# netty/netty

Hardware: AMD Instinct MI355X
Metric: GiB/s device-resident Snappy encode+decode, 64 KiB chunks, 1/2/4/8 MI355X (higher is better)
Workload: dtype u8; 1 GPU; configs[4]: Snappy encode (+frame CRC32C) then decode + CRC32C verify of 1638400 text-like 64 KiB chunks (100 GiB) split across 1 GPU(s), device-resident; chunk_bytes=65536, global_chunks=1638400, chunks_per_gpu=1638400, parallelism=dp1 (independent chunk shards, no data-path collective)

## Files before the change

### netty_amd/csrc/snappy_encode.hip

```cpp
#include <stdlib.h>
#include <algorithm>
#include <mutex>
#include <vector>
#include "nx_common.hpp"
#include "workspace.hpp"

namespace nx {
namespace enc {

typedef uint32_t __attribute__((aligned(1))) u32u;

typedef uint64_t __attribute__((aligned(1))) u64u;

__device__ __forceinline__ uint32_t ld32(const uint8_t* p) { return *reinterpret_cast<const u32u*>(p); }
__device__ __forceinline__ uint64_t ld64(const uint8_t* p) { return *reinterpret_cast<const u64u*>(p); }
__device__ __forceinline__ uint32_t hash_of(uint32_t le, int shift) {
    return (__builtin_bswap32(le) * 0x1e35a7bdu) >> shift;
}

template <bool PAIR>
struct WriterT {
    uint32_t* w;
    uint32_t acc;
    uint32_t na;
    uint32_t nw;
    uint32_t s0;
    __device__ __forceinline__ void emit(uint32_t v) {
        if (!PAIR) {
            w[nw] = v;
        } else if (nw & 1u) {
            *reinterpret_cast<uint2*>(w + nw - 1u) = make_uint2(s0, v);
        } else {
            s0 = v;
        }
        ++nw;
    }
    __device__ __forceinline__ void put(uint32_t b) {
        acc |= b << (8 * na);
        if (++na == 4) {
            emit(acc);
            acc = 0;
            na = 0;
        }
    }
    __device__ __forceinline__ void copy(const uint8_t* p, int32_t n) {
        while (n >= 4) {
            const uint32_t v = ld32(p);
            if (na == 0) {
                emit(v);
            } else {
                emit(acc | (v << (8 * na)));
                acc = v >> (32 - 8 * na);
            }
            p += 4;
            n -= 4;
        }
        while (n-- > 0) put(*p++);
    }
    __device__ __forceinline__ uint32_t pos() const { return nw * 4 + na; }
    __device__ __forceinline__ void finish() {
        if (PAIR && (nw & 1u)) w[nw - 1u] = s0;
        uint8_t* t = reinterpret_cast<uint8_t*>(w + nw);
        for (uint32_t i = 0; i < na; ++i) t[i] = (uint8_t)(acc >> (8 * i));
    }
};

template <int SD>
struct WriterL {
    uint32_t* st;
    uint32_t* dst;
    uint32_t acc;
    uint32_t na;
    uint32_t nw;
    uint32_t s;
    uint32_t lo;
    __device__ __forceinline__ WriterL(uint32_t* stage, uint8_t* o)
        : st(stage), dst(reinterpret_cast<uint32_t*>(o)), acc(0), na(0), nw(0) {
        s = (uint32_t)(((uintptr_t)o >> 2) & (SD - 1));
        lo = s;
    }
    __device__ __forceinline__ void emit(uint32_t v) {
        st[s] = v;
        ++nw;
        if (s == SD - 1) {
            uint32_t* g = dst + nw - SD;
            if (lo == 0) {
#pragma unroll
                for (int q = 0; q < SD / 4; ++q)
                    reinterpret_cast<uint4*>(g)[q] = make_uint4(st[4 * q], st[4 * q + 1], st[4 * q + 2], st[4 * q + 3]);
            } else {
                for (uint32_t j = lo; j < SD; ++j) g[j] = st[j];
                lo = 0;
            }
            s = 0;
        } else {
            ++s;
        }
    }
    __device__ __forceinline__ void put(uint32_t b) {
        acc |= b << (8 * na);
        if (++na == 4) {
            emit(acc);
            acc = 0;
            na = 0;
        }
    }
    __device__ __forceinline__ void copy(const uint8_t* p, int32_t n) {
        while (n >= 4) {
            const uint32_t v = ld32(p);
            if (na == 0) {
                emit(v);
            } else {
                emit(acc | (v << (8 * na)));
                acc = v >> (32 - 8 * na);
            }
            p += 4;
            n -= 4;
        }
        while (n-- > 0) put(*p++);
    }
    __device__ __forceinline__ uint32_t pos() const { return nw * 4 + na; }
    __device__ __forceinline__ void finish() {
        uint32_t* g = dst + nw - s;
        for (uint32_t j = lo; j < s; ++j) g[j] = st[j];
        uint8_t* t = reinterpret_cast<uint8_t*>(dst + nw);
        for (uint32_t i = 0; i < na; ++i) t[i] = (uint8_t)(acc >> (8 * i));
    }
};

struct ByteWriter {
    uint8_t* o;
    uint32_t n;
    __device__ __forceinline__ void put(uint32_t b) { o[n++] = (uint8_t)b; }
    __device__ __forceinline__ void copy(const uint8_t* p, int32_t k) {
        for (int32_t i = 0; i < k; ++i) o[n + i] = p[i];
        n += (uint32_t)k;
    }
    __device__ __forceinline__ uint32_t pos() const { return n; }
    __device__ __forceinline__ void finish() {}
};

template <class Wr>
__device__ __forceinline__ void enc_literal(const uint8_t* in, Wr& w, int32_t length) {
    if (length < 61) {
        w.put((uint32_t)((length - 1) << 2));
    } else {
        const int32_t v = length - 1;
        const int bitLength = 31 - __clz((uint32_t)v);
        const int bytesToEncode = 1 + bitLength / 8;
        w.put((uint32_t)((59 + bytesToEncode) << 2));
        for (int i = 0; i < bytesToEncode; i++) w.put((uint32_t)((v >> (i * 8)) & 0xff));
    }
    w.copy(in, length);
}

template <class Wr>
__device__ __forceinline__ void enc_copy_off(Wr& w, int32_t offset, int32_t length) {
    if (length < 12 && offset < 2048) {
        w.put((uint32_t)(1 | ((length - 4) << 2) | ((offset >> 8) << 5)));
        w.put((uint32_t)(offset & 0xff));
    } else {
        w.put((uint32_t)(2 | ((length - 1) << 2)));
        w.put((uint32_t)(offset & 0xff));
        w.put((uint32_t)((offset >> 8) & 0xff));
    }
}

template <class Wr>
__device__ __forceinline__ void enc_copy(Wr& w, int32_t offset, int32_t length) {
    while (length >= 68) {
        enc_copy_off(w, offset, 64);
        length -= 64;
    }
    if (length > 64) {
        enc_copy_off(w, offset, 60);
        length -= 60;
    }
    enc_copy_off(w, offset, length);
}

struct StreamWin {
    const uint8_t* origin;
    uint32_t pad;
    uint32_t end;
    uint32_t wb;
    uint32_t w0, w1, w2, w3, w4, w5, w6, w7;
    uint32_t f0, f1, f2, f3;
    __device__ __forceinline__ void init(const uint8_t* in, int32_t length) {
        pad = (uint32_t)((uintptr_t)in & 15u);
        origin = in - pad;
        end = pad + (uint32_t)length;
        wb = 0x80000000u;
    }
    __device__ __forceinline__ static uint32_t sel(uint32_t i, uint32_t a0, uint32_t a1, uint32_t a2, uint32_t a3, uint32_t a4,
                                                   uint32_t a5, uint32_t a6, uint32_t a7) {
        const bool b0 = i & 1u, b1 = i & 2u, b2 = i & 4u;
        const uint32_t c0 = b0 ? a1 : a0, c1 = b0 ? a3 : a2, c2 = b0 ? a5 : a4, c3 = b0 ? a7 : a6;
        const uint32_t d0 = b1 ? c1 : c0, d1 = b1 ? c3 : c2;
        return b2 ? d1 : d0;
    }
    __device__ __forceinline__ uint32_t get(int32_t p) {
        const uint32_t q = (uint32_t)p + pad;
        uint32_t off = q - wb;
        if (off > 27u) {
            if (off < 44u) {
                wb += 16u;
                w0 = w4; w1 = w5; w2 = w6; w3 = w7;
                w4 = f0; w5 = f1; w6 = f2; w7 = f3;
                if (wb + 32u < end) {
                    const uint4 z = *reinterpret_cast<const uint4*>(origin + wb + 32u);
                    f0 = z.x; f1 = z.y; f2 = z.z; f3 = z.w;
                }
            } else {
                wb = q & ~15u;
                const uint4 x = *reinterpret_cast<const uint4*>(origin + wb);
                w0 = x.x; w1 = x.y; w2 = x.z; w3 = x.w;
                if (wb + 16u < end) {
                    const uint4 y = *reinterpret_cast<const uint4*>(origin + wb + 16u);
                    w4 = y.x; w5 = y.y; w6 = y.z; w7 = y.w;
                }
                if (wb + 32u < end) {
                    const uint4 z = *reinterpret_cast<const uint4*>(origin + wb + 32u);
                    f0 = z.x; f1 = z.y; f2 = z.z; f3 = z.w;
                }
            }
            off = q - wb;
        }
        const uint32_t i = off >> 2;
        const uint32_t lo = sel(i, w0, w1, w2, w3, w4, w5, w6, w7);
        const uint32_t hi = sel(i + 1u, w0, w1, w2, w3, w4, w5, w6, w7);
        return __builtin_amdgcn_alignbyte(hi, lo, off & 3u);
    }
};

__device__ __forceinline__ uint64_t ld_cand(const uint8_t* in, int32_t c, int32_t length) {
    return c + 8 <= length ? ld64(in + c) : (uint64_t)ld32(in + c);
}

__device__ __forceinline__ int32_t match_len(const uint8_t* in, StreamWin& win, int32_t a, int32_t b, int32_t length,
                                             uint32_t first) {
    int32_t m = 0;
    if (b <= length - 4) {
        const uint32_t x0 = first ^ win.get(b);
        if (x0) return (int32_t)(__builtin_ctz(x0) >> 3);
        m = 4;
        while (b + m <= length - 4) {
            const uint32_t x = ld32(in + a + m) ^ win.get(b + m);
            if (x) return m + (int32_t)(__builtin_ctz(x) >> 3);
            m += 4;
        }
    }
    while (b + m < length && in[a + m] == in[b + m]) ++m;
    return m;
}

template <bool SWAP, class Wr>
__device__ uint32_t encode_chunk(const uint8_t* __restrict__ in, int32_t length, Wr& w, uint32_t* __restrict__ table, uint32_t stamp) {
    for (int i = 0;; i++) {
        const uint32_t b = (uint32_t)length >> (i * 7);
        if ((b & 0xFFFFFF80u) != 0) {
            w.put((b & 0x7f) | 0x80);
        } else {
            w.put(b);
            break;
        }
    }
    uint32_t hts = length <= 1 ? 1u : (1u << (32 - __clz((uint32_t)(length - 1))));
    if (hts > 16384u) hts = 16384u;
    const int shift = __clz(hts) + 1;
    const uint32_t stag = stamp << 28;
    const uint32_t word0 = length >= 4 ? ld32(in) : 0u;
#define TST(ptr, v) (*(ptr) = (v))
#define XCH(ptr, v) (SWAP ? __hip_atomic_exchange((ptr), (v), __ATOMIC_RELAXED, __HIP_MEMORY_SCOPE_AGENT) \
                          : ({ const uint32_t o_ = *(ptr); *(ptr) = (v); o_; }))
#define CHK(wd) (((wd) ^ ((wd) >> 12) ^ ((wd) >> 24)) & 0xFFFu)
#define MK(pos, wd) (stag | (CHK(wd) << 16) | (uint32_t)(pos))
#define LIVE(e) (((e) & 0xF0000000u) == stag)
#define TBL_DEC(e) (LIVE(e) ? (int32_t)((e) & 0xFFFFu) : 0)
#define MAYBE(e, wd) (LIVE(e) ? ((((e) >> 16) & 0xFFFu) == CHK(wd)) : ((wd) == word0))
    int32_t nextEmit = 0;
    if (length >= 15) {
        StreamWin win;
        win.init(in, length);
        int32_t inIndex = 1;
        uint32_t nextWord = win.get(1);
        uint32_t nextHash = hash_of(nextWord, shift);
        for (;;) {
            int32_t skip = 32;
            int32_t nextIndex = inIndex;
            int32_t candidate;
            uint32_t curWord;
            uint64_t cand8;
            uint32_t entry;
            do {
                inIndex = nextIndex;
                const uint32_t hash = nextHash;
                curWord = nextWord;
                nextIndex = inIndex + (skip++ >> 5);
                if (nextIndex > length - 4) goto done;
                nextWord = win.get(nextIndex);
                nextHash = hash_of(nextWord, shift);
                entry = XCH(table + hash, MK(inIndex, curWord));
                candidate = TBL_DEC(entry);
            } while (!(MAYBE(entry, curWord) && curWord == (uint32_t)(cand8 = ld_cand(in, candidate, length))));

            enc_literal(in + nextEmit, w, inIndex - nextEmit);

            int32_t insertTail;
            for (;;) {
                const int32_t base = inIndex;
                const int32_t matched = 4 + match_len(in, win, candidate + 4, inIndex + 4, length, (uint32_t)(cand8 >> 32));
                inIndex += matched;
                enc_copy(w, base - candidate, matched);
                insertTail = inIndex - 1;
                nextEmit = inIndex;
                if (inIndex >= length - 4) goto done;
                const uint32_t wTail = win.get(insertTail);
                const uint32_t wCur = win.get(inIndex);
                const uint32_t prevHash = hash_of(wTail, shift);
                TST(table + prevHash, MK(inIndex - 1, wTail));
                const uint32_t currentHash = hash_of(wCur, shift);
                const uint32_t e = XCH(table + currentHash, MK(inIndex, wCur));
                candidate = TBL_DEC(e);
                if (!MAYBE(e, wCur) || wCur != (uint32_t)(cand8 = ld_cand(in, candidate, length))) break;
            }
            nextWord = win.get(insertTail + 2);
            nextHash = hash_of(nextWord, shift);
            ++inIndex;
        }
    }
done:
#undef TBL_DEC
#undef MAYBE
#undef LIVE
#undef MK
#undef CHK
#undef XCH
#undef TST
    if (nextEmit < length) enc_literal(in + nextEmit, w, length - nextEmit);
    w.finish();
    return w.pos();
}

__device__ __forceinline__ uint32_t bytes_at(const uint8_t* in, int32_t p, int32_t length) {
    if (p + 4 <= length) return ld32(in + p);
    uint32_t v = 0;
    for (int32_t i = 0; p + i < length && i < 4; ++i) v |= (uint32_t)in[p + i] << (8 * i);
    return v;
}

__device__ __forceinline__ int32_t match_len_w(const uint8_t* in, StreamWin& win, int32_t a, int32_t b, int32_t length, uint32_t cn3) {
    int32_t m = 0;
    if (b <= length - 4) {
        const uint32_t x0 = (cn3 ^ win.get(b)) & 0xFFFFFFu;
        if (x0) return (int32_t)(__builtin_ctz(x0) >> 3);
        m = 3;
        while (b + m <= length - 4) {
            const uint32_t x = ld32(in + a + m) ^ win.get(b + m);
            if (x) return m + (int32_t)(__builtin_ctz(x) >> 3);
            m += 4;
        }
    }
    while (b + m < length && in[a + m] == in[b + m]) ++m;
    return m;
}

template <class Wr>
__device__ uint32_t encode_chunk_w(const uint8_t* __restrict__ in, int32_t length, Wr& w, uint64_t* __restrict__ table, uint32_t stamp) {
    for (int i = 0;; i++) {
        const uint32_t b = (uint32_t)length >> (i * 7);
        if ((b & 0xFFFFFF80u) != 0) {
            w.put((b & 0x7f) | 0x80);
        } else {
            w.put(b);
            break;
        }
    }
    uint32_t hts = length <= 1 ? 1u : (1u << (32 - __clz((uint32_t)(length - 1))));
    if (hts > 16384u) hts = 16384u;
    const int shift = __clz(hts) + 1;
    int32_t nextEmit = 0;
    if (length >= 15) {
        const uint32_t pbits = hts == 16384u ? 16u : (uint32_t)(32 - shift);
        const uint32_t pmask = (1u << pbits) - 1u, rmask = (1u << shift) - 1u;
        const uint64_t stag = (uint64_t)stamp << 58;
        const uint32_t word0 = ld32(in);
        const uint32_t n3_0 = bytes_at(in, 4, length) & 0xFFFFFFu;
#define RES(wd) ((__builtin_bswap32(wd) * 0x1e35a7bdu) & rmask)
#define MKW(pos, wd, n3) (stag | ((uint64_t)(n3) << 34) | ((uint64_t)RES(wd) << pbits) | (uint64_t)(uint32_t)(pos))
#define WLIVE(e) ((uint32_t)((e) >> 58) == stamp)
#define WMATCH(e, wd) (WLIVE(e) ? (((uint32_t)((e) >> pbits) & rmask) == RES(wd)) : ((wd) == word0))
#define WPOS(e) (WLIVE(e) ? (int32_t)((uint32_t)(e) & pmask) : 0)
#define WN3(e) (WLIVE(e) ? ((uint32_t)((e) >> 34) & 0xFFFFFFu) : n3_0)
#define XCH64(ptr, v) __hip_atomic_exchange((ptr), (v), __ATOMIC_RELAXED, __HIP_MEMORY_SCOPE_AGENT)
        StreamWin win;
        win.init(in, length);
        int32_t inIndex = 1;
        uint32_t nextWord = win.get(1);
        uint32_t nextHash = hash_of(nextWord, shift);
        for (;;) {
            int32_t skip = 32;
            int32_t nextIndex = inIndex;
            uint64_t entry;
            uint32_t curWord;
            do {
                inIndex = nextIndex;
                const uint32_t hash = nextHash;
                curWord = nextWord;
                nextIndex = inIndex + (skip++ >> 5);
                if (nextIndex > length - 4) goto done;
                const uint32_t n3 = win.get(inIndex + 4) & 0xFFFFFFu;
                nextWord = win.get(nextIndex);
                nextHash = hash_of(nextWord, shift);
                entry = XCH64(table + hash, MKW(inIndex, curWord, n3));
            } while (!WMATCH(entry, curWord));
            int32_t candidate = WPOS(entry);
            uint32_t cn3 = WN3(entry);

            enc_literal(in + nextEmit, w, inIndex - nextEmit);

            int32_t insertTail;
            for (;;) {
                const int32_t base = inIndex;
                const int32_t matched = 4 + match_len_w(in, win, candidate + 4, inIndex + 4, length, cn3);
                inIndex += matched;
                enc_copy(w, base - candidate, matched);
                insertTail = inIndex - 1;
                nextEmit = inIndex;
                if (inIndex >= length - 4) goto done;
                const uint32_t wTail = win.get(insertTail);
                const uint32_t wCur = win.get(inIndex);
                const uint32_t n3c = win.get(inIndex + 4) & 0xFFFFFFu;
                const uint32_t n3t = ((wCur >> 24) | (n3c << 8)) & 0xFFFFFFu;
                const uint32_t prevHash = hash_of(wTail, shift);
                __hip_atomic_store(table + prevHash, MKW(inIndex - 1, wTail, n3t), __ATOMIC_RELAXED, __HIP_MEMORY_SCOPE_AGENT);
                const uint32_t currentHash = hash_of(wCur, shift);
                const uint64_t e = XCH64(table + currentHash, MKW(inIndex, wCur, n3c));
                if (!WMATCH(e, wCur)) break;
                candidate = WPOS(e);
                cn3 = WN3(e);
            }
            nextWord = win.get(insertTail + 2);
            nextHash = hash_of(nextWord, shift);
            ++inIndex;
        }
#undef XCH64
#undef WN3
#undef WPOS
#undef WMATCH
#undef WLIVE
#undef MKW
#undef RES
    }
done:
    if (nextEmit < length) enc_literal(in + nextEmit, w, length - nextEmit);
    w.finish();
    return w.pos();
}

constexpr int kStageDw = 16;
template <bool SWAP, bool SPREAD>
__global__ void __launch_bounds__(256, 5) k_snappy_encode(const uint8_t* __restrict__ in, const uint64_t* __restrict__ in_off,
                                                       const uint32_t* __restrict__ in_len, uint8_t* __restrict__ out,
                                                       const uint64_t* __restrict__ out_off, uint32_t* __restrict__ out_len,
                                                       int32_t* __restrict__ status, uint32_t n, uint64_t* __restrict__ workspace,
                                                       uint32_t stamp_base) {
    const uint32_t gtid = blockIdx.x * blockDim.x + threadIdx.x;
    if (SPREAD && (gtid & 63u) != 0u) return;
    const uint32_t tid = SPREAD ? gtid >> 6 : gtid;
    const uint32_t nthreads = SPREAD ? (gridDim.x * blockDim.x) >> 6 : gridDim.x * blockDim.x;
    uint64_t* table = workspace + (size_t)tid * 16384u;
    uint32_t* stage = nullptr;
    if constexpr (!SPREAD) {
        __shared__ uint32_t stages[256 * (kStageDw + 1)];
        stage = &stages[threadIdx.x * (kStageDw + 1)];
    }
    uint32_t iter = 0;
    for (uint32_t c = tid; c < n; c += nthreads, ++iter) {
        const uint32_t len = in_len[c];
        if (len > 65536u) {
            status[c] = NX_ERR_INVALID_ARG;
            out_len[c] = 0;
            continue;
        }
        const uint32_t stamp = stamp_base + iter + 1u;
        uint8_t* o = out + out_off[c];
        uint32_t olen;
        const uint8_t* src = in + in_off[c];
        if (!SPREAD && (((uintptr_t)o) & 3u) == 0) {
            WriterL<kStageDw> w(stage, o);
            olen = encode_chunk_w(src, (int32_t)len, w, table, stamp);
        } else if ((((uintptr_t)o) & 7u) == 0) {
            WriterT<true> w{reinterpret_cast<uint32_t*>(o), 0, 0, 0, 0};
            olen = encode_chunk_w(src, (int32_t)len, w, table, stamp);
        } else if ((((uintptr_t)o) & 3u) == 0) {
            WriterT<false> w{reinterpret_cast<uint32_t*>(o), 0, 0, 0, 0};
            olen = encode_chunk_w(src, (int32_t)len, w, table, stamp);
        } else {
            ByteWriter w{o, 0};
            olen = encode_chunk_w(src, (int32_t)len, w, table, stamp);
        }
        out_len[c] = olen;
        status[c] = NX_OK;
    }
}

constexpr uint32_t kLdsTableBytes = 16384u * 4u;
constexpr uint32_t kLdsBytes = kLdsTableBytes + 65536u + 16u;
__global__ void __launch_bounds__(64) k_snappy_encode_lds(const uint8_t* __restrict__ in, const uint64_t* __restrict__ in_off,
                                                         const uint32_t* __restrict__ in_len, uint8_t* __restrict__ out,
                                                         const uint64_t* __restrict__ out_off, uint32_t* __restrict__ out_len,
                                                         int32_t* __restrict__ status, uint32_t n) {
    extern __shared__ __attribute__((aligned(16))) uint8_t smem[];
    uint32_t* table = reinterpret_cast<uint32_t*>(smem);
    uint8_t* buf = smem + kLdsTableBytes;
    const uint32_t t = threadIdx.x;
    for (uint32_t c = blockIdx.x; c < n; c += gridDim.x) {
        const uint32_t len = in_len[c];
        if (len > 65536u) {
            if (t == 0) {
                status[c] = NX_ERR_INVALID_ARG;
                out_len[c] = 0;
            }
            continue;
        }
        const uint8_t* src = in + in_off[c];
        for (uint32_t i = t; i < 16384u / 4u; i += 64u) reinterpret_cast<uint4*>(table)[i] = make_uint4(0, 0, 0, 0);
        for (uint32_t i = 4u * t; i < len; i += 256u) {
            uint32_t v = 0;
            if (i + 4u <= len) {
                v = ld32(src + i);
            } else {
                for (uint32_t k = 0; i + k < len; ++k) v |= (uint32_t)src[i + k] << (8 * k);
            }
            *reinterpret_cast<uint32_t*>(buf + i) = v;
        }
        __syncthreads();
        if (t == 0) {
            uint8_t* o = out + out_off[c];
            uint32_t olen;
            if ((((uintptr_t)o) & 7u) == 0) {
                WriterT<true> w{reinterpret_cast<uint32_t*>(o), 0, 0, 0, 0};
                olen = encode_chunk<false>(buf, (int32_t)len, w, table, 1u);
            } else if ((((uintptr_t)o) & 3u) == 0) {
                WriterT<false> w{reinterpret_cast<uint32_t*>(o), 0, 0, 0, 0};
                olen = encode_chunk<false>(buf, (int32_t)len, w, table, 1u);
            } else {
                ByteWriter w{o, 0};
                olen = encode_chunk<false>(buf, (int32_t)len, w, table, 1u);
            }
            out_len[c] = olen;
            status[c] = NX_OK;
        }
        __syncthreads();
    }
}

}
}

namespace {
constexpr unsigned kEncBlock = 256;
constexpr uint32_t kMaxStamp = 63;
static_assert(nx::kWsSpec[(int)nx::WsKind::SnappyEnc].entry_bytes == sizeof(uint64_t) &&
                  nx::kWsSpec[(int)nx::WsKind::SnappyEnc].lg == 14 && nx::kWsSpec[(int)nx::WsKind::SnappyEnc].waves_per_cu == 20,
              "Snappy table geometry: 16384 64-bit entries, 20 waves per CU");
}

namespace {
constexpr size_t kEncTableBytes = 16384u * sizeof(uint64_t);

size_t enc_plan(size_t n, size_t slots, int cus, uint32_t* sizes, size_t cap) {
    auto put = [&](size_t i, size_t v) {
        if (sizes && i < cap) sizes[i] = (uint32_t)v;
    };
    if (n == 0) return 0;
    if (n <= slots) {
        put(0, n);
        return 1;
    }
    const size_t k = (n + slots - 1) / slots;
    const size_t G = (size_t)cus * 128u;
    const size_t s = n / k / G * G;
    const size_t rem = n - k * s, plus = rem / G, last = rem - plus * G;
    if (s > 0 && (plus == 0 || s + G <= slots) && s + last <= slots) {
        for (size_t i = 0; i < k; ++i) put(i, s + (i < plus ? G : 0) + (i + 1 == k ? last : 0));
        return k;
    }
    const size_t e = (n + k - 1) / k;
    for (size_t i = 0; i < k; ++i) put(i, std::min(e, n - i * e));
    return k;
}
}

extern "C" int32_t nx_snappy_encoder_reserve_ex(uint32_t max_chunks, uint64_t max_bytes, void* stream, uint64_t* bytes, uint64_t* peak) {
    int dev = 0, cus = 256;
    NX_HIP_CHECK(hipGetDevice(&dev));
    NX_HIP_CHECK(hipDeviceGetAttribute(&cus, hipDeviceAttributeMultiprocessorCount, dev));
    if (bytes) *bytes = 0;
    if (peak) *peak = 0;
    nx::SharedWs& W = nx::shared_ws(nx::WsKind::SnappyEnc, dev);
    uint32_t units = max_chunks;
    if (max_bytes) {
        size_t lanes = (size_t)(max_bytes / kEncTableBytes);
        if (lanes > nx::kSpreadMaxChunks) lanes = lanes / 256 * 256;
        if (lanes == 0) return NX_ERR_INVALID_ARG;
        std::lock_guard<std::mutex> lk(W.mu);
        if (W.p && W.slots > lanes) return NX_ERR_INVALID_ARG;
        W.cap = lanes;
        if (units > lanes) units = (uint32_t)lanes;
    }
    if (max_chunks <= (uint32_t)cus) return NX_OK;
    const int32_t r = nx::ws_hold(nx::WsKind::SnappyEnc, dev, units, (hipStream_t)stream);
    if (r != NX_OK) return r;
    {
        std::lock_guard<std::mutex> lk(W.mu);
        W.kept = true;
        if (bytes) *bytes = (uint64_t)W.slots * kEncTableBytes;
        if (peak) *peak = W.place.peak;
    }
    nx::ws_unhold(nx::WsKind::SnappyEnc, dev);
    return NX_OK;
}

extern "C" int32_t nx_snappy_encoder_reserve(uint32_t max_chunks, void* stream) {
    return nx_snappy_encoder_reserve_ex(max_chunks, 0, stream, nullptr, nullptr);
}

extern "C" int32_t nx_snappy_encode_plan_for(uint32_t n, uint32_t slots, int32_t cus, uint32_t* sizes, uint32_t cap, uint32_t* count) {
    if (!count || (cap && !sizes) || slots == 0 || cus <= 0) return NX_ERR_INVALID_ARG;
    *count = (uint32_t)enc_plan(n, slots, cus, sizes, cap);
    return NX_OK;
}

extern "C" int32_t nx_snappy_encode_plan(uint32_t n, uint32_t* sizes, uint32_t cap, uint32_t* count) {
    if (!count || (cap && !sizes)) return NX_ERR_INVALID_ARG;
    int dev = 0, cus = 256;
    NX_HIP_CHECK(hipGetDevice(&dev));
    NX_HIP_CHECK(hipDeviceGetAttribute(&cus, hipDeviceAttributeMultiprocessorCount, dev));
    *count = 0;
    if (n == 0) return NX_OK;
    if (n <= (uint32_t)cus) {
        if (cap) sizes[0] = n;
        *count = 1;
        return NX_OK;
    }
    nx::SharedWs& W = nx::shared_ws(nx::WsKind::SnappyEnc, dev);
    std::lock_guard<std::mutex> lk(W.mu);
    const size_t want = nx::ws_capped(W, nx::ws_want(nx::WsKind::SnappyEnc, n, cus));
    const size_t have = W.p && W.slots >= want ? W.slots : std::max(want, W.p ? W.slots : (size_t)0);
    const nx::LaneGrid g = nx::ws_grid(nx::WsKind::SnappyEnc, n, cus, have);
    if (g.spread) {
        if (cap) sizes[0] = n;
        *count = 1;
        return NX_OK;
    }
    *count = (uint32_t)enc_plan(n, g.slots, cus, sizes, cap);
    return NX_OK;
}

extern "C" int32_t nx_snappy_encode_batch(const uint8_t* in, const uint64_t* in_off, const uint32_t* in_len, uint8_t* out,
                                          const uint64_t* out_off, uint32_t* out_len, int32_t* status, uint32_t n, void* stream) {
    NX_CLEAR_STALE_ERROR();
    if (n == 0) return NX_OK;
    if (!in || !in_off || !in_len || !out || !out_off || !out_len || !status) return NX_ERR_INVALID_ARG;
    int dev = 0, cus = 256;
    NX_HIP_CHECK(hipGetDevice(&dev));
    NX_HIP_CHECK(hipDeviceGetAttribute(&cus, hipDeviceAttributeMultiprocessorCount, dev));
    const hipStream_t st = (hipStream_t)stream;
    if (n <= (uint32_t)cus) {
        static std::once_flag once;
        static hipError_t attr = hipSuccess;
        std::call_once(once, [] {
            attr = hipFuncSetAttribute((const void*)nx::enc::k_snappy_encode_lds, hipFuncAttributeMaxDynamicSharedMemorySize,
                                       (int)nx::enc::kLdsBytes);
        });
        NX_HIP_CHECK(attr);
        hipLaunchKernelGGL(nx::enc::k_snappy_encode_lds, dim3(n), dim3(64), nx::enc::kLdsBytes, st, in, in_off, in_len, out, out_off,
                           out_len, status, n);
        NX_HIP_CHECK(hipGetLastError());
        return NX_OK;
    }
    nx::WsLease lease(nx::WsKind::SnappyEnc, dev, st);
    NX_HIP_CHECK(lease.acquire(nx::ws_want(nx::WsKind::SnappyEnc, n, cus)));
    nx::SharedWs& W = lease.ws();
    const nx::LaneGrid g = nx::ws_grid(nx::WsKind::SnappyEnc, n, cus, W.slots);
    uint64_t* ws = static_cast<uint64_t*>(W.p);
    auto stamps = [&](uint32_t iters) -> hipError_t {
        if (W.stamp + iters < kMaxStamp) return hipSuccess;
        W.stamp = 0;
        return hipMemsetAsync(ws, 0, W.slots * kEncTableBytes, st);
    };
    if (g.spread) {
        const size_t per_launch = g.slots * (kMaxStamp - 1);
        for (size_t base = 0; base < n; base += per_launch) {
            const uint32_t m = (uint32_t)std::min<size_t>(per_launch, n - base);
            const uint32_t iters = (uint32_t)((m + g.slots - 1) / g.slots);
            NX_HIP_CHECK(stamps(iters));
            const size_t waves = std::min<size_t>(g.slots, m);
            hipLaunchKernelGGL((nx::enc::k_snappy_encode<true, true>), dim3((unsigned)waves), dim3(64), 0, st, in, in_off + base,
                               in_len + base, out, out_off + base, out_len + base, status + base, m, ws, W.stamp);
            NX_HIP_CHECK(hipGetLastError());
            W.stamp += iters;
        }
        return NX_OK;
    }
    const size_t k = enc_plan(n, g.slots, cus, nullptr, 0);
    std::vector<uint32_t> sizes(k);
    enc_plan(n, g.slots, cus, sizes.data(), k);
    size_t base = 0;
    for (size_t i = 0; i < k; ++i) {
        const uint32_t m = sizes[i];
        NX_HIP_CHECK(stamps(1));
        hipLaunchKernelGGL((nx::enc::k_snappy_encode<true, false>), dim3((m + kEncBlock - 1) / kEncBlock), dim3(kEncBlock), 0, st, in,
                           in_off + base, in_len + base, out, out_off + base, out_len + base, status + base, m, ws, W.stamp);
        NX_HIP_CHECK(hipGetLastError());
        W.stamp += 1;
        base += m;
    }
    return NX_OK;
}

extern "C" int32_t nx_snappy_encode_placement(float* probe_ms, int32_t cap, int32_t* n, int32_t* pick) {
    if (!n || !pick || (cap > 0 && !probe_ms)) return NX_ERR_INVALID_ARG;
    int dev = 0;
    NX_HIP_CHECK(hipGetDevice(&dev));
    nx::SharedWs& W = nx::shared_ws(nx::WsKind::SnappyEnc, dev);
    std::lock_guard<std::mutex> lk(W.mu);
    *n = W.place.n;
    *pick = W.place.pick;
    for (int32_t k = 0; k < W.place.n && k < cap; ++k) probe_ms[k] = W.place.ms[k];
    return NX_OK;
}
```

Before: 52.66 GiB/s.

## Prefetch encoder input window into LDS via async global_load_lds staging

Adds a StageWin sliding window for the dense per-thread Snappy encoder that prefetches the next 32 input bytes into a per-thread LDS slot with global_load_lds, so sequential window advances read from LDS instead of issuing dependent global loads. The window type is chosen at compile time (default StageWin for the non-spread kernel) and threaded through encode_chunk_w and match_len_w. This aims to hide global-load latency in the hash-scan loop. In exchange it adds LDS usage, which can reduce occupancy, plus explicit waitcnt stalls that may serialize the loop.

Result: no change. 53.06 GiB/s, median of 6 (+0.7%).

```diff
diff --git a/netty_amd/csrc/snappy_encode.hip b/netty_amd/csrc/snappy_encode.hip
--- a/netty_amd/csrc/snappy_encode.hip
+++ b/netty_amd/csrc/snappy_encode.hip
@@ -229,6 +229,62 @@
         const uint32_t i = off >> 2;
         const uint32_t lo = sel(i, w0, w1, w2, w3, w4, w5, w6, w7);
         const uint32_t hi = sel(i + 1u, w0, w1, w2, w3, w4, w5, w6, w7);
+        return __builtin_amdgcn_alignbyte(hi, lo, off & 3u);
+    }
+};
+
+struct StageWin {
+    const uint8_t* origin;
+    uint32_t pad;
+    uint32_t end;
+    uint32_t wb;
+    uint32_t w0, w1, w2, w3, w4, w5, w6, w7;
+    uint32_t* row;
+    __device__ __forceinline__ void bind(uint32_t* stages) { row = stages + (threadIdx.x >> 6) * 512u; }
+    __device__ __forceinline__ void init(const uint8_t* in, int32_t length) {
+        pad = (uint32_t)((uintptr_t)in & 31u);
+        origin = in - pad;
+        end = pad + (uint32_t)length;
+        wb = 0x80000000u;
+    }
+    __device__ __forceinline__ void fill(uint32_t s) {
+        typedef const __attribute__((address_space(1))) void* gptr;
+        typedef __attribute__((address_space(3))) void* lptr;
+        const uint8_t* g = origin + s;
+        asm volatile("s_waitcnt lgkmcnt(0)" ::: "memory");
+        __builtin_amdgcn_global_load_lds((gptr)g, (lptr)row, 16, 0, 0);
+        __builtin_amdgcn_global_load_lds((gptr)(g + 16), (lptr)(row + 256), 16, 0, 0);
+    }
+    __device__ __forceinline__ uint32_t get(int32_t p) {
+        const uint32_t q = (uint32_t)p + pad;
+        uint32_t off = q - wb;
+        if (off > 27u) {
+            if (off < 44u) {
+                wb += 16u;
+                w0 = w4; w1 = w5; w2 = w6; w3 = w7;
+                const uint32_t nb = wb + 16u;
+                const uint4 z = *reinterpret_cast<const uint4*>(row + (threadIdx.x & 63u) * 4u + ((nb & 16u) ? 256u : 0u));
+                w4 = z.x; w5 = z.y; w6 = z.z; w7 = z.w;
+                if ((nb & 16u) && nb + 16u < end) fill(nb + 16u);
+            } else {
+                wb = q & ~15u;
+                const uint4 x = *reinterpret_cast<const uint4*>(origin + wb);
+                w0 = x.x; w1 = x.y; w2 = x.z; w3 = x.w;
+                if (wb + 16u < end) {
+                    const uint4 y = *reinterpret_cast<const uint4*>(origin + wb + 16u);
+                    w4 = y.x; w5 = y.y; w6 = y.z; w7 = y.w;
+                }
+                const uint32_t s = (wb + 32u) & ~31u;
+                if (s < end) {
+                    asm volatile("s_waitcnt vmcnt(0)" ::: "memory");
+                    fill(s);
+                }
+            }
+            off = q - wb;
+        }
+        const uint32_t i = off >> 2;
+        const uint32_t lo = StreamWin::sel(i, w0, w1, w2, w3, w4, w5, w6, w7);
+        const uint32_t hi = StreamWin::sel(i + 1u, w0, w1, w2, w3, w4, w5, w6, w7);
         return __builtin_amdgcn_alignbyte(hi, lo, off & 3u);
     }
 };
@@ -349,7 +405,8 @@
     return v;
 }
 
-__device__ __forceinline__ int32_t match_len_w(const uint8_t* in, StreamWin& win, int32_t a, int32_t b, int32_t length, uint32_t cn3) {
+template <class Win>
+__device__ __forceinline__ int32_t match_len_w(const uint8_t* in, Win& win, int32_t a, int32_t b, int32_t length, uint32_t cn3) {
     int32_t m = 0;
     if (b <= length - 4) {
         const uint32_t x0 = (cn3 ^ win.get(b)) & 0xFFFFFFu;
@@ -365,8 +422,9 @@
     return m;
 }
 
-template <class Wr>
-__device__ uint32_t encode_chunk_w(const uint8_t* __restrict__ in, int32_t length, Wr& w, uint64_t* __restrict__ table, uint32_t stamp) {
+template <class Win, class Wr>
+__device__ uint32_t encode_chunk_w(const uint8_t* __restrict__ in, int32_t length, Wr& w, uint64_t* __restrict__ table, uint32_t stamp,
+                                   Win& win) {
     for (int i = 0;; i++) {
         const uint32_t b = (uint32_t)length >> (i * 7);
         if ((b & 0xFFFFFF80u) != 0) {
@@ -393,7 +451,6 @@
 #define WPOS(e) (WLIVE(e) ? (int32_t)((uint32_t)(e) & pmask) : 0)
 #define WN3(e) (WLIVE(e) ? ((uint32_t)((e) >> 34) & 0xFFFFFFu) : n3_0)
 #define XCH64(ptr, v) __hip_atomic_exchange((ptr), (v), __ATOMIC_RELAXED, __HIP_MEMORY_SCOPE_AGENT)
-        StreamWin win;
         win.init(in, length);
         int32_t inIndex = 1;
         uint32_t nextWord = win.get(1);
@@ -459,6 +516,28 @@
 }
 
 constexpr int kStageDw = 16;
+constexpr int kInStageDw = 8;
+#ifndef NX_ENC_DENSE_WIN
+#define NX_ENC_DENSE_WIN StageWin
+#endif
+template <class W>
+struct IsStaged {
+    static constexpr bool value = false;
+};
+template <>
+struct IsStaged<StageWin> {
+    static constexpr bool value = true;
+};
+template <bool SPREAD>
+struct WinOf {
+    typedef NX_ENC_DENSE_WIN type;
+    static constexpr bool staged = IsStaged<NX_ENC_DENSE_WIN>::value;
+};
+template <>
+struct WinOf<true> {
+    typedef StreamWin type;
+    static constexpr bool staged = false;
+};
 template <bool SWAP, bool SPREAD>
 __global__ void __launch_bounds__(256, 5) k_snappy_encode(const uint8_t* __restrict__ in, const uint64_t* __restrict__ in_off,
                                                        const uint32_t* __restrict__ in_len, uint8_t* __restrict__ out,
@@ -471,9 +550,14 @@
     const uint32_t nthreads = SPREAD ? (gridDim.x * blockDim.x) >> 6 : gridDim.x * blockDim.x;
     uint64_t* table = workspace + (size_t)tid * 16384u;
     uint32_t* stage = nullptr;
+    typename WinOf<SPREAD>::type win;
     if constexpr (!SPREAD) {
         __shared__ uint32_t stages[256 * (kStageDw + 1)];
         stage = &stages[threadIdx.x * (kStageDw + 1)];
+        if constexpr (WinOf<SPREAD>::staged) {
+            __shared__ __attribute__((aligned(16))) uint32_t in_stages[256 * kInStageDw];
+            win.bind(in_stages);
+        }
     }
     uint32_t iter = 0;
     for (uint32_t c = tid; c < n; c += nthreads, ++iter) {
@@ -489,16 +573,16 @@
         const uint8_t* src = in + in_off[c];
         if (!SPREAD && (((uintptr_t)o) & 3u) == 0) {
             WriterL<kStageDw> w(stage, o);
-            olen = encode_chunk_w(src, (int32_t)len, w, table, stamp);
+            olen = encode_chunk_w(src, (int32_t)len, w, table, stamp, win);
         } else if ((((uintptr_t)o) & 7u) == 0) {
             WriterT<true> w{reinterpret_cast<uint32_t*>(o), 0, 0, 0, 0};
-            olen = encode_chunk_w(src, (int32_t)len, w, table, stamp);
+            olen = encode_chunk_w(src, (int32_t)len, w, table, stamp, win);
         } else if ((((uintptr_t)o) & 3u) == 0) {
             WriterT<false> w{reinterpret_cast<uint32_t*>(o), 0, 0, 0, 0};
-            olen = encode_chunk_w(src, (int32_t)len, w, table, stamp);
+            olen = encode_chunk_w(src, (int32_t)len, w, table, stamp, win);
         } else {
             ByteWriter w{o, 0};
-            olen = encode_chunk_w(src, (int32_t)len, w, table, stamp);
+            olen = encode_chunk_w(src, (int32_t)len, w, table, stamp, win);
         }
         out_len[c] = olen;
         status[c] = NX_OK;
```
